# neofytr/LLMTokenizer

Measured on AMD Instinct MI355X. Metric: corpus MB/s per merge iter (train), 1 GiB synthetic corpus, higher is better.
Workload: dtype u32

## Files before the change

### llmtokenizer_amd/csrc/batch.hip

```cpp
#pragma once
#include "engine_common.h"

namespace bpeamd {

static_assert(TOPK == 64, "a wave holds a list, one entry per lane");
static_assert(BRB == 2 * (1024 / 64), "the select's 16 waves merge two partial lists each");
#ifndef BPE_SU
#define BPE_SU 1
#endif
#ifndef BPE_FORM_PRINT
#define BPE_FORM_PRINT 0
#endif
#ifndef BPE_RU
#define BPE_RU 4
#endif
#ifndef BPE_AU
#define BPE_AU 1
#endif
constexpr uint32_t AU = BPE_AU;
constexpr uint32_t SU = BPE_SU;
#ifndef BPE_RUN_THREAD_PAIRS
#define BPE_RUN_THREAD_PAIRS 16
#endif
constexpr uint32_t RUN_THREAD_PAIRS = BPE_RUN_THREAD_PAIRS, RUN_Q = 256;
// ... 819 lines not shown
        B->ticket = 0;
        B->k = k;
        B->z0 = 256 + md;
        nmem = k;
    }
    ts_mark(E, bi, BT_SEL_FOLD, false);
    __syncthreads();
    if (tid < nmem) E->tlen[256 + sc.merges_done + tid] = ctl[tid];
    for (uint32_t q = tid; q < CTL_SELECT_WORDS; q += blockDim.x) reinterpret_cast<uint32_t *>(Cg)[q] = scw[q];
    if (tid == 0) {
        Cg->hot_scanned = sc.hot_scanned;
        if (sc.err) Cg->err = sc.err;
    }
    for (uint32_t q = tid; q < BAT_HEAD_WORDS; q += blockDim.x) reinterpret_cast<uint32_t *>(Bg)[q] = sbw[q];
    for (uint32_t q = tid; q < clear_k * 4; q += blockDim.x) E->bvnl[q] = 0;
    if (xclr_k) {
        if (tid < XBH) E->xbat[tid] = 0;
        if (tid < 2 * xclr_k) E->xbat[XBH + (uint64_t)(tid >> 1) * xbat_member_words(xclr_w) + (tid & 1)] = 0;
    }
    if (tid == 0 && sc.stop != STOP_NONE && E->hprobe) {
        __hip_atomic_store(E->hprobe, sc.stop, __ATOMIC_RELAXED, __HIP_MEMORY_SCOPE_SYSTEM);
        __builtin_amdgcn_fence(__ATOMIC_RELEASE, "");
    }
    ts_mark(E, bi, BT_SEL_WB, false);
    ts_mark(E, bi, BT_SEL_OUT, false, true);
}

__device__ inline void rewrite_occ(const Eng *__restrict__ E, Ctl *__restrict__ C, Bat *__restrict__ B, uint32_t z,
                                   uint32_t la, uint32_t lb, uint32_t base, uint32_t obase, uint32_t elo, uint32_t ehi,
                                   uint32_t bidm, uint32_t nbm, uint64_t L1) {
    uint32_t *tok = E->tok;
    const uint64_t n = E->n0;
    const uint32_t tid = threadIdx.x;
    for (uint32_t e0 = elo + bidm * blockDim.x * RU; e0 < ehi; e0 += nbm * blockDim.x * RU) {
        uint32_t pos[RU];
        uint16_t tg[RU];
#pragma unroll
        for (uint32_t u = 0; u < RU; u++) {
            const uint32_t e = e0 + u * blockDim.x + tid;
            pos[u] = e < ehi ? E->ids_out[base + e] : 0u;
            tg[u] = e < ehi ? E->btag[base + e] : (uint16_t)0;
        }
#pragma unroll
        for (uint32_t u = 0; u < RU; u++) {
            const uint32_t e = e0 + u * blockDim.x + tid;
            if (e >= ehi) continue;
            const uint64_t i = pos[u], j = i + la, kq = j + lb;
            tok[i] = z;
            if (j < n) {
                if (kq - 1 - i > E->end_max) B->ra_err = 5;
                if (kq - 1 == j) {
                    tok[j] = end_code(kq - 1 - i);
                } else {
                    tok[j] = HOLE;
                    if (kq - 1 < n) tok[kq - 1] = end_code(kq - 1 - i);
                }
                if (j == L1) C->L1new = (uint32_t)i;
            }
            E->occ[obase + e] = (uint32_t)i;
            E->occnb[obase + e] = tg[u];
        }
    }
}

__device__ __attribute__((always_inline)) inline void bat_rewrite(const Eng *__restrict__ E, Ctl *__restrict__ C, Bat *__restrict__ B) {
    __shared__ uint32_t sz[BK], sla[BK], slb[BK], sR[BK], slo[BK], ssb[BK], spre[BK + 1], ablk[BK + 1];
    __shared__ uint32_t sk, stop_, am, last;
    const uint32_t tid = threadIdx.x, lane = tid & 63;
    const uint32_t nA = gridDim.x - BRB, bid = blockIdx.x - BRB;
    if (tid < 64) {
        const uint32_t k = aload(&B->ra_k);
        uint32_t R[NBK], lo[NBK], nb[NBK], nbp[NBK];
        unsigned long long tot = 0;
#pragma unroll
        for (uint32_t b = 0; b < NBK; b++) {
            const uint32_t q = 64 * b + lane;
            const bool in = q < k;
            R[b] = in ? B->ra_R[q] : 0u;
            lo[b] = in ? B->ra_lo[q] : 0u;
            tot += R[b] - lo[b];
        }
        tot = wave_sum(tot);
#pragma unroll
        for (uint32_t b = 0; b < NBK; b++) {
            const uint32_t q = 64 * b + lane;
            nb[b] = q < k ? 1 + (uint32_t)(tot ? (uint64_t)(nA - k) * (R[b] - lo[b]) / tot : 0) : 0;
            nbp[b] = nb[b];
        }
// ... 211 lines not shown
__device__ inline uint32_t tok_at_b(const uint32_t *__restrict__ tok, const BHalo &H, int64_t p, int64_t n) {
    if (p < 0) return SH && p >= -3 ? get3(H.HL, (uint32_t)(-1 - p)) : HOLE;
    if (p >= n) return SH && p - n < 3 ? get3(H.HR, (uint32_t)(p - n)) : HOLE;
    return tok[p];
}

template <bool SH>
__device__ inline uint32_t cover_of(const uint32_t *__restrict__ tok, const RoleTab &rt, const BHalo &H, uint32_t p,
                                    int64_t ps, int64_t n) {
    if (!(rt.get(p) >> 31)) return BK;
    const int64_t pps = v_left<SH>(tok, ps);
    const uint32_t pp = tok_at_b<SH>(tok, H, pps, n);
    const uint32_t mm = rt.member(pp, p);
    if (mm >= BK || pp != p) return mm;
    uint32_t L;
    if (SH && ps < 0) {
        L = H.hlr[mm];
    } else {
        L = 1;
        int64_t x = v_left<SH>(tok, ps);
        for (; x >= 0 && tok[x] == p; x = v_left<SH>(tok, x)) L++;
        if (SH && x < 0) L += H.hlr[mm];
    }
    return (L & 1) ? BK : mm;
}

template <bool SH>
__device__ inline uint32_t starts_of(const uint32_t *__restrict__ tok, const RoleTab &rt, const BHalo &H, uint32_t q,
                                     int64_t kq, int64_t n) {
    const uint32_t lq = rt.get(q) & 0x7FFFFFFFu;
    if (!lq) return BK;
    const int64_t kn = v_right(kq, lq, n);
    return rt.member(q, tok_at_b<SH>(tok, H, kn, n));
}

enum : uint32_t { GRF_LGO = 1, GRF_LEND = 2, GRF_IGO = 3, GRF_IEND = 4 };
__device__ void bscan_long_runs(const Eng *__restrict__ E, Bat *__restrict__ B, const uint32_t *__restrict__ tok,
                                const RoleTab &rt, const BHalo &H, int64_t n, uint32_t z0, uint32_t sgen) {
    const uint32_t lane = threadIdx.x & 63;
    const uint32_t ng = uni(min(aload(&B->gr_n), GRUN));
    const uint64_t stride = gr_stride(E->n0), maxch = stride - 1;
    auto flag_of = [&](uint32_t st) { return (sgen << 3) | st; };
    for (uint32_t gi = 0; gi < ng; gi++) {
        uint32_t ok = 1;
        if (lane == 0) {
            const unsigned long long t0 = wall_clock64();
            while (__hip_atomic_load(&B->gr_ready[gi], __ATOMIC_ACQUIRE, __HIP_MEMORY_SCOPE_AGENT) != sgen) {
                if (wall_clock64() - t0 > E->gr_wait) {
                    ok = 0;
                    B->ra_err = 11;
                    atomicAdd(&B->gr_tready, 1u);
                    break;
                }
                __builtin_amdgcn_s_sleep(1);
            }
        }
        if (!uni((uint32_t)__shfl((int)ok, 0))) return;
        const uint32_t mg = uni(aload(&B->gr_m[gi])), ag = uni(B->a[mg]), zg = z0 + mg;
        const int64_t c0 = uni(aload(&B->gr_c[gi])), lag = uni(E->tlen[ag]);
        uint32_t *occg = E->ids_out + B->sbase[mg];
        uint16_t *tagg = E->btag + B->sbase[mg];
        const uint32_t slice = B->sbase[mg + 1] - B->sbase[mg];
        uint32_t *flags = E->grflag + (uint64_t)gi * stride;
        auto pos = [&](int64_t l) -> int64_t { return c0 + l * lag; };
        auto tk = [&](int64_t l) -> uint32_t {
            const int64_t p = pos(l);
// ... 189 lines not shown
        if (SH) {
            Halo h;
            shard_halo(E->erec, E->nshards, E->shard, sa[tid], &h);
            H.hlr[tid] = h.hlrun;
            H.myi[tid] = h.myidx;
            if (tid == 0)
                for (int q = 0; q < 3; q++) {
                    H.HL[q] = h.HL[q];
                    H.HR[q] = h.HR[q];
                }
        }
    }
    const uint32_t a = sa[m], b = sb[m], z = z0 + m;
    const uint32_t la = E->tlen[a], lb = E->tlen[b];
    const uint32_t mode = B->mode[m], off = B->off[m], len = B->len[m];
    const uint32_t bid = blockIdx.x - B->blk0[m], nblk = B->blk0[m + 1] - B->blk0[m];
    const uint32_t sbase = B->sbase[m];
    uint32_t *occz = E->ids_out + sbase;
    uint16_t *tagz = E->btag + sbase;
    const uint32_t sslice = B->sbase[m + 1] - sbase;
#define STG(IDX, WHERE) if ((IDX) >= sslice) { B->ra_err = 12; } else
    uint32_t *Rm = &B->R[m];
    const int64_t n = (int64_t)E->n0;
    const uint32_t *__restrict__ tok = E->tok;
    const uint32_t want = mode == 2 ? a : b;
    const uint32_t lim = min(DENSE, z0 + k);
    for (uint32_t v = 0; v < 4; v++)
        for (uint32_t x = tid; x < lim; x += SCAN_T) s[v][x] = 0;
    __syncthreads();
    auto tok_at = [&](int64_t p) -> uint32_t { return tok_at_b<SH>(tok, H, p, n); };

    if (a != b) {
        static_assert(SU == 1 && BPE_WFLUSH, "the wave-driven candidate loop: one entry per lane per round");
        const uint32_t stride = nblk * SCAN_T;
        const uint32_t lane = tid & 63, wbase = (tid >> 6) * 64 * FR;
        uint32_t wcnt = 0, wocc = 0;
        uint32_t nent[SU];
        uint16_t ntg[SU];
        uint32_t eS = bid * SCAN_T + (tid & ~63u);
        auto load1 = [&](uint32_t s0, uint32_t &en, uint16_t &tg) {
            const uint32_t e = s0 + lane;
            en = 0;
            tg = 0xFFFFu;
            if (e < len) {
                en = mode == 0 ? E->plist[off + e] : E->occ[off + e];
                if (mode) tg = E->occnb[off + e];
            }
        };
        uint32_t pent = 0;
        uint16_t ptg = 0xFFFFu;
        auto advance = [&]() {
            eS += stride;
            if (SCAN_PD > 1) {
                nent[0] = pent;
                ntg[0] = ptg;
                if (eS + stride < len) load1(eS + stride, pent, ptg);
            } else if (eS < len) {
                load1(eS, nent[0], ntg[0]);
            }
        };
        auto flush = [&]() {
            __builtin_amdgcn_fence(__ATOMIC_RELEASE, "wavefront");
            __builtin_amdgcn_wave_barrier();
            uint32_t g = 0;
            if (lane == 0 && wcnt) g = atomicAdd(Rm, wcnt);
            g = __shfl(g, 0);
            for (uint32_t q = lane; q < wcnt; q += 64) {
                STG(g + q, "wflush") {
                occz[g + q] = list[wbase + q];
                tagz[g + q] = ltag[wbase + q];
                }
            }
            wocc += wcnt;
            wcnt = 0;
            __builtin_amdgcn_wave_barrier();
        };
        const bool cmp = mode != 0 && E->scan_compact != 0;
        const uint32_t tsh = mode == 2 ? 8u : 0u;
        uint32_t qpos = 0, qn = 0;
        load1(eS, nent[0], ntg[0]);
        if (SCAN_PD > 1) load1(eS + stride, pent, ptg);
        for (;;) {
            uint32_t ent[SU];
            uint16_t etg[SU];
            bool val[SU];
            if (!cmp) {
                if (eS >= len) break;
                val[0] = eS + lane < len;
                ent[0] = nent[0];
                etg[0] = ntg[0];
                advance();
            } else {
                while (eS < len) {
                    const bool pass = eS + lane < len && tag_ok(((uint32_t)ntg[0] >> tsh) & 0xFFu, want);
                    const unsigned long long M = __ballot(pass);
                    const uint32_t np = (uint32_t)__popcll(M);
                    if (qn + np > 64) break;
                    const uint32_t r = lane - qn;
                    const bool mine = lane >= qn && r < np;
                    const uint32_t pv = (uint32_t)__shfl((int)nent[0], (int)(mine ? kth_bit(M, r) : lane));
                    if (mine) qpos = pv;
                    qn += np;
                    advance();
                }
                if (qn == 0) break;
                val[0] = lane < qn;
                ent[0] = qpos;
                etg[0] = 0xFFFFu;
                qn = 0;
            }
            int64_t ii[SU], jj[SU];
            TokWin W[SU];
#pragma unroll
            for (uint32_t u = 0; u < SU; u++) {
                if (mode == 2) {
                    val[u] = val[u] && tag_ok(etg[u] >> 8, want);
                    jj[u] = ent[u];
                    ii[u] = 0;
                    if (val[u]) W[u] = tok_window(tok, jj[u]);
                } else {
                    val[u] = val[u] && (mode == 0 || tag_ok(etg[u] & 0xFFu, want));
                    ii[u] = ent[u];
                    jj[u] = ii[u] + la;
                    if (val[u]) W[u] = tok_window(tok, ii[u]);
                }
            }
            bool ok[SU];
            uint32_t tl[SU], tr[SU];
#pragma unroll
            for (uint32_t u = 0; u < SU; u++) {
                ok[u] = false;
                tl[u] = tr[u] = HOLE;
                if (!val[u]) continue;
                const int64_t j = jj[u];
                if (mode == 2) {
                    const uint32_t wl = j > 0 ? W[u].at(j - 1) : HOLE;
                    const int64_t i = j > 0 ? start_of_end<SH>(wl, j - 1) : -1;
                    ii[u] = i;
                    if (W[u].at(j) != b || i < 0) continue;
                    const uint32_t ti = W[u].has(i) ? W[u].at(i) : tok[i];
                    tl[u] = i > 0 ? (W[u].has(i - 1) ? W[u].at(i - 1) : tok[i - 1]) : HOLE;
                    const int64_t kk = j + lb;
                    tr[u] = kk < n ? (W[u].has(kk) ? W[u].at(kk) : tok[kk]) : HOLE;
                    ok[u] = ti == a;
                } else {
                    const int64_t i = ii[u], kk = j + lb;
                    const uint32_t t1 = j >= n ? HOLE : W[u].has(j) ? W[u].at(j) : tok[j];
                    tl[u] = i > 0 ? W[u].at(i - 1) : HOLE;
                    tr[u] = kk >= n ? HOLE : W[u].has(kk) ? W[u].at(kk) : tok[kk];
                    ok[u] = W[u].at(i) == a && t1 == b && j < n;
                }
            }
            int64_t ps[SU];
            uint32_t pv[SU];
#pragma unroll
            for (uint32_t u = 0; u < SU; u++) {
                const int64_t i = ii[u];
                ps[u] = i <= 0 ? -1 : start_of_end<SH>(tl[u], i - 1);
                pv[u] = ok[u] ? ((i > 0 && is_id(tl[u])) ? tl[u] : tok_at(ps[u])) : HOLE;
            }
#pragma unroll
            for (uint32_t u = 0; u < SU; u++) {
                const int64_t i = ii[u], j = jj[u];
                uint32_t lfin = HOLE, rfin = HOLE;
                if (ok[u]) {
                    const uint32_t p = pv[u];
                    lfin = p;
                    if (p != HOLE) {
                        const uint32_t cv = cover_of<SH>(tok, rt, H, p, ps[u], n);
                        if (cv < BK) {
                            lfin = z0 + cv;
                            mk_set(tadj, cv);
                            atomicAdd(&covc, 1u);
                        } else {
                            vadd_b(s, E, m, V_DL, p, gcnt);
                            vadd_b(s, E, m, V_IL, p, gcnt);
                        }
                    }
                    const int64_t kq = v_right(j, lb, n);
                    const uint32_t q = kq < n ? tr[u] : tok_at(kq);
                    rfin = q;
                    if (q != HOLE) {
                        const uint32_t st = starts_of<SH>(tok, rt, H, q, kq, n);
                        if (st < BK) {
                            rfin = z0 + st;
                            mk_set(tadj, st);
                        }
                        vadd_b(s, E, m, V_DR, q, gcnt);
                        vadd_b(s, E, m, V_IR, rfin, gcnt);
                    }
                }
                const unsigned long long om = __ballot(ok[u]);
                if (ok[u]) {
                    const uint32_t slot = wbase + wcnt + (uint32_t)__popcll(om & ((1ull << lane) - 1ull));
                    list[slot] = (uint32_t)i;
                    ltag[slot] = nb_tag(lfin, rfin);
                }
                wcnt += (uint32_t)__popcll(om);
            }
            if (wcnt + 64 > 64 * FR) flush();
        }
        if (wcnt) flush();
        if (lane == 0 && wocc) atomicAdd(&bRs, wocc);
    } else {
        for (uint32_t e0 = bid * SCAN_T; e0 < len; e0 += nblk * SCAN_T) {
            const uint32_t e = e0 + tid;
            int64_t i = 0;
            bool ok = false;
            if (e >= len) {
            } else if (mode == 2) {
                const int64_t j = E->occ[off + e];
                if (tag_ok(E->occnb[off + e] >> 8, want) && tok[j] == b) {
                    i = v_left<SH>(tok, j);
                    ok = i >= 0 && tok[i] == a;
                }
            } else {
                i = (mode == 0) ? E->plist[off + e] : E->occ[off + e];
                ok = (mode == 0 || tag_ok(E->occnb[off + e] & 0xFFu, want)) && tok[i] == a && i + la < n &&
                     tok[i + la] == b;
            }
            const int64_t ps = ok ? v_left<SH>(tok, i) : -1;
            const uint32_t p = ok ? tok_at(ps) : HOLE;
            const uint32_t cv = (ok && p != HOLE && p != a) ? cover_of<SH>(tok, rt, H, p, ps, n) : BK;
            if (cv < BK) {
                atomicAdd(&covc, 1u);
                mk_set(tadj, cv);
// ... 941 lines not shown
```

### llmtokenizer_amd/csrc/encode.hip

```cpp

namespace bpeamd {

__device__ inline void enc_desc(const Eng *E, uint32_t u, uint32_t v, uint32_t z, uint32_t *mode, uint32_t *off,
                                uint32_t *len) {
    *mode = 1;
    *off = 0;
    *len = 0;
    if (!(u < z && v < z)) return;
    if (u < 256 && v < 256) {
        const uint32_t ru = E->rank[u], rv = E->rank[v];
        if (ru != HOLE && rv != HOLE) {
            const uint32_t rk = ru * E->A + rv;
            *mode = 0;
            *off = E->poff[rk];
            *len = E->poff[rk + 1] - *off;
        }
        return;
    }
    if (u >= v) {
        *off = E->occ_off[u];
        *len = E->occ_len[u];
    } else {
        *mode = 2;
        *off = E->occ_off[v];
// ... 295 lines not shown
            C->counters[5] += spre[nb];
            C->counters[6]++;
            C->n_live -= spre[nb];
            const uint32_t xl = SH ? C->xleft : HOLE;
            if (xl != HOLE) {
                const uint64_t end = (uint64_t)xl + C->xleft_lb;
                if (end - 1 == xl) {
                    tok[xl] = MARKV;
                } else {
                    tok[xl] = HOLE;
                    if (end - 1 < n) tok[end - 1] = MARKV;
                }
                C->F1 = (uint32_t)(end < n ? end : n);
            }
        }
        __syncthreads();
        form_batch(E, C, E->eb + (p ^ 1), C->merges_done, occ_base + spre[nb]);
        return;
    }
    const uint32_t total = sseg[nb];
    const uint32_t *scratch = E->ids_out;
    const uint32_t nw = gridDim.x - 1;
    const uint64_t L1 = SH ? C->L1 : 0;
    for (uint32_t t = blockIdx.x * blockDim.x + tid; t < total; t += nw * blockDim.x) {
        const uint32_t m = seg_of(sseg, nb, t);
        const uint32_t q = t - sseg[m];
        if (q >= sR[m]) continue;
        const uint64_t i = scratch[t];
        const uint64_t j = i + sla[m], k = j + slb[m];
        tok[i] = sz[m];
        if (!SH || j < n) {
            if (k - 1 - i > E->end_max) C->err = 5;
            if (k - 1 == j) {
                tok[j] = end_code(k - 1 - i);
            } else {
                tok[j] = HOLE;
                if (!SH || k - 1 < n) tok[k - 1] = end_code(k - 1 - i);
            }
            if (SH && j == L1) C->L1new = (uint32_t)i;
        }
        E->occ[occ_base + spre[m] + q] = (uint32_t)i;
    }
}

template <bool SH>
__global__ __launch_bounds__(256) void k_link_batch(const Eng *__restrict__ E, const Ctl *__restrict__ C) {
    if (C->stop) return;
    const EncBatch *B = E->eb + C->ebp;
    const uint32_t nb = B->nbg;
    __shared__ uint32_t sseg[BMAX + 1], sz[BMAX], sR[BMAX], spre[BMAX + 1];
    const uint32_t tid = threadIdx.x;
    for (uint32_t m = tid; m <= nb; m += blockDim.x) sseg[m] = B->seg[m];
    for (uint32_t m = tid; m < nb; m += blockDim.x) {
        sz[m] = B->z[m];
        sR[m] = B->R[m];
    }
    __syncthreads();
    block_exscan256(sR, spre, nb);
    const uint32_t total = sseg[nb], occ_base = B->occ_base;
    const int64_t n = (int64_t)E->n0;
    const uint32_t *tok = E->tok;
    for (uint32_t t = blockIdx.x * blockDim.x + tid; t < total; t += gridDim.x * blockDim.x) {
        const uint32_t m = seg_of(sseg, nb, t);
        const uint32_t q = t - sseg[m];
        if (q >= sR[m]) continue;
        const uint32_t e = occ_base + spre[m] + q;
        const int64_t i = E->occ[e];
        const int64_t ps = v_left<SH>(tok, i);
        const int64_t k = i + E->tlen[sz[m]];
        E->occnb[e] = nb_tag(ps >= 0 ? tok[ps] : HOLE, k < n ? tok[k] : HOLE);
// ... 10 lines not shown
```

### llmtokenizer_amd/csrc/engine.hip

```cpp
#include <hip/hip_runtime.h>
#include <fcntl.h>
#include <unistd.h>
#include <cerrno>

#include <algorithm>
#include <chrono>
#include <cstdio>
#include <cstdlib>
#include <cstring>
#include <string>
#include <thread>
#include <vector>
#include <unordered_map>

#include <rocprim/rocprim.hpp>

#include "../../include/bpe_gpu.h"
#include "kernels.hip"
#include "batch.hip"
#include "encode.hip"
#include "encode_win.hip"
#include "encode_docs.hip"
#include "split.hip"
#include "train_split.hip"
// ... 437 lines not shown
    if (r) {
        c->zpend.clear();
        return r;
    }
    return 0;
}

int setup_run_body(bpe_gpu_ctx *c, uint32_t mcap, bool encode) {
    free_train(c);
    if (!encode) c->split_ready = false;
    Eng &h = c->h;
    h.n0 = c->n0;
    h.mcap = mcap;
    h.vcap = 256 + mcap;
    h.encode = encode ? 1 : 0;
    h.fast = c->fast || c->sharded;
    h.sharded = c->sharded;
    h.shard = c->shard;
    h.nshards = c->nshards;
    const uint64_t n0 = c->n0;
    int r;
    if ((r = dalloc(c, &h.tok, n0 + 8, false))) return r;
    if ((r = dalloc(c, &h.tlen, h.vcap))) return r;
    if ((r = dalloc(c, &h.rank, 256))) return r;
    if ((r = dalloc(c, &h.plist, n0, false))) return r;
    const uint64_t slack = c->sharded ? std::max<uint64_t>((uint64_t)mcap + 64, n0 / 16) : 0;
    const uint64_t occ_n = (n0 + slack + 2) & ~1ull;
    if ((r = dalloc(c, &h.occ, occ_n + n0, false))) return r;
    h.ids_out = h.occ + occ_n;
    if ((r = dalloc(c, &h.occnb, occ_n, false))) return r;
    h.xfused = c->sharded && c->xfused && !encode;
    h.end_max = END_MAX;
    if (const char *t = getenv("BPE_END_MAX")) h.end_max = std::min<uint64_t>(END_MAX, std::max(1ll, atoll(t)));
    h.track_ub = 1;
    if (const char *t = getenv("BPE_TRACK")) h.track_ub = (uint32_t)std::min(2, std::max(0, atoi(t)));
    h.light_wait = 100000000ull;
    if (const char *t = getenv("BPE_LIGHT_WAIT_TICKS")) h.light_wait = strtoull(t, nullptr, 10);
    h.xtimeout = c->xtimeout;
    h.xstride = (uint32_t)(((4ull * h.vcap + 2) + 63) & ~63ull);
    if (c->sharded) {
        if ((r = dalloc(c, &h.xbuf, 2ull * h.xstride))) return r;
        if ((r = dalloc(c, &h.myrec, EDGE_WORDS))) return r;
        if ((r = dalloc(c, &h.erec, (size_t)EDGE_WORDS * c->nshards))) return r;
    } else {
        h.xbuf = h.myrec = h.erec = nullptr;
    }
    if ((r = dalloc(c, &h.occ_off, h.vcap))) return r;
    if ((r = dalloc(c, &h.occ_len, h.vcap))) return r;
    if ((r = dalloc(c, &h.merges, 2ull * std::max<uint32_t>(mcap, 1)))) return r;
    for (int p = 0; p < 2; p++) {
        for (int v = 0; v < 4; v++) {
            if ((r = dalloc(c, &h.vec[p][v], encode ? 1 : std::max<uint32_t>(h.vcap, DENSE)))) return r;
            if ((r = dalloc(c, &h.vlist[p][v], encode ? 1 : h.vcap, false))) return r;
        }
        if ((r = dalloc(c, &h.vnl[p], 4))) return r;
    }
    if ((r = dalloc(c, &h.vecd, encode ? 1 : (size_t)2 * REPL * 4 * DENSE))) return r;
    if ((r = dalloc(c, &h.scan_tend, STAMPS))) return r;
    h.dbgts = nullptr;
    h.dbg_form = (uint32_t)getenv_int("BPE_DEBUG_FORM", 0);
    h.prefix_apply = (uint32_t)(getenv_int("BPE_PREFIX", 1) != 0);
    {
        int khz = 0;
        (void)hipDeviceGetAttribute(&khz, hipDeviceAttributeWallClockRate, c->dev);
        const int us = getenv_int("BPE_RW_HOLD_US", 0);
        h.rw_hold = (uint32_t)std::max(0, us) * (uint32_t)std::max(1, khz / 1000);
// ... 3164 lines not shown
```

### llmtokenizer_amd/csrc/engine_common.h

```cpp
#pragma once
#include <hip/hip_runtime.h>
#include <stddef.h>
#include <stdint.h>

namespace bpeamd {

constexpr uint32_t HOLE = 0xFFFFFFFFu;
constexpr uint32_t END_FLAG = 0x80000000u;
constexpr uint32_t MARKV = 0xFFFFFFFEu;
constexpr uint64_t END_MAX = 0x7FFFFFFDull;
__host__ __device__ inline bool is_id(uint32_t v) { return v < END_FLAG; }
__host__ __device__ inline uint32_t end_code(uint64_t d) { return END_FLAG | (uint32_t)d; }
#ifndef BPE_DENSE
#define BPE_DENSE 8192
#endif
constexpr uint32_t DENSE = BPE_DENSE;
#ifndef BPE_REPL
#define BPE_REPL 8
#endif
constexpr uint32_t REPL = BPE_REPL;
constexpr uint32_t NTHR = 16;
constexpr uint64_t CHUNK = 65536;
constexpr uint64_t DYN_LIMIT = CHUNK * NTHR;
constexpr uint64_t TRACK_LIMIT = 2 * DYN_LIMIT;
constexpr uint64_t TRACK_MIN_N = 4096;
constexpr uint64_t MERGED_B0 = 65536;
constexpr uint64_t THREAD_B0 = 256;
constexpr uint32_t L1W = 1024;
constexpr uint32_t L2W = 256;
constexpr uint32_t EDGE_WORDS = 16;
constexpr uint32_t TS_SLOTS = 16384;
enum { TS_K1_IN = 0, TS_K1_RESCAN, TS_K1_SCAN, TS_K2_IN, TS_K2_SELECT, TS_K2_APPLY_A, TS_K2_APPLY_B, TS_K1_LASTIN,
       TS_S_CAND, TS_S_LIST, TS_S_DELTA, TS_B_DVAL, TS_B_TABLE, TS_B_MARKS, TS_B_PROBE, TS_B_COUNT, TS_K1_CLEARED,
       TS_SPARE0, TS_SPARE1, TS_SPARE2, TS_SPARE3, TS_SPARE4, TS_SPARE5, TS_SPARE6, TS_SPARE7, TS_SPARE8, TS_N };

enum { V_DL = 0, V_DR = 1, V_IL = 2, V_IR = 3 };

enum : uint32_t {
    STOP_NONE = 0,
    STOP_DONE = 1,
    STOP_CAP = 2,
    STOP_EVENT = 3,
    STOP_GROW = 4,
    STOP_ERROR = 5,
    STOP_ENC_END = 6,
// ... 180 lines not shown
    const uint32_t *enc_pairs;
    uint32_t n_enc;
    EncBatch *eb;
    uint32_t hot;
    uint32_t hot_parts;
    uint32_t hot_target;
    uint32_t relist_stale;
    uint32_t *hot_slot;
    uint32_t *hot_hist;
    unsigned long long *hotp_best, *hotp_key, *hotp_v2, *hotp_k2;
    uint32_t *hotp_tie;
    uint32_t batch;
    uint32_t skip_on;
    uint32_t scan_compact;
    uint32_t scan_occd;
    uint32_t skg_exp;
    uint32_t nlists;
    uint32_t tie_up;
    uint32_t crate_pct;
    uint32_t lose_retry;
    uint32_t bvs;
    Bat *bat;
    uint16_t *btag;
    uint32_t *bvecd;
    uint32_t *bvec;
    uint32_t *bvlist;
    uint32_t *bvnl;
    uint32_t *xbat;
    uint32_t *grflag;
    unsigned long long gr_wait;
    uint32_t *xsp_out, *xsp_in;
    uint32_t xsp_cap, xsp_stride;
    uint64_t end_max;
    uint32_t track_ub;
    unsigned long long light_wait;
    unsigned long long *lkey, *lfirst;
    uint64_t lcap;
    unsigned long long *mlog;
    uint64_t mlog_cap;
};
constexpr uint32_t MLOG_WORDS = 5;
constexpr uint64_t MLOG_MAX = 1ull << 20;

struct Ctl {
    uint32_t a, b, z, stop;
    uint32_t merges_done, parity, R, occ_top;
    uint32_t cand_mode, cand_off, cand_len, stop_z;
    uint32_t nl2, full, event, ties;
    unsigned long long n_live;
    unsigned long long D;
    unsigned long long B;
    unsigned long long W;
    uint32_t edge, wslot, pad0, pad1;
    unsigned long long Bcur[NTHR];
    unsigned long long Bstart[NTHR];
    unsigned long long Bfin[NTHR];
    uint32_t Dt[NTHR];
    uint32_t follows[NTHR];
    uint32_t last_c[NTHR];
    unsigned long long stat_n;
    unsigned long long counters[12];
    unsigned long long scan_t0;
    unsigned long long scan_ticks;
    unsigned long long scan_launches;
    uint32_t sa, sb, s_mode, s_off;
    uint32_t s_len, spec, sRp[2];
// ... 166 lines not shown
```

### llmtokenizer_amd/csrc/kernels.hip

```cpp
#include "engine_common.h"
#include "p2p.hip"

namespace bpeamd {

__device__ inline uint32_t lane_id() { return __lane_id(); }

__device__ inline uint32_t aload(const uint32_t *p) {
    return __hip_atomic_load(p, __ATOMIC_RELAXED, __HIP_MEMORY_SCOPE_AGENT);
}
__device__ inline void astore(uint32_t *p, uint32_t v) {
    __hip_atomic_store(p, v, __ATOMIC_RELAXED, __HIP_MEMORY_SCOPE_AGENT);
}
__device__ inline unsigned long long aload64(const unsigned long long *p) {
    return __hip_atomic_load(p, __ATOMIC_RELAXED, __HIP_MEMORY_SCOPE_AGENT);
}

__device__ inline uint32_t wave_append(bool pred, uint32_t *counter) {
    unsigned long long m = __ballot(pred);
    if (m == 0) return 0;
    uint32_t lane = lane_id();
    uint32_t leader = __ffsll(m) - 1;
    uint32_t base = 0;
    if (lane == leader) base = atomicAdd(counter, (uint32_t)__popcll(m));
    base = __shfl(base, leader);
// ... 38 lines not shown
            atomicOr(&C->err, P2P_ERR_BIT);
            break;
        }
        __builtin_amdgcn_s_sleep(1);
    }
}

struct LazyHalo {
    const Eng *E;
    Ctl *C;
    uint32_t a;
    bool wait;
    bool ready;
    Halo h;
    __device__ inline const Halo &get() {
        if (!ready) {
            if (wait) {
                wait_records(E, C);
                shard_halo_ld(E->erec, E->nshards, E->shard, a, &h, [](const uint32_t *q) { return aload(q); });
            } else {
                shard_halo(E->erec, E->nshards, E->shard, a, &h);
            }
            ready = true;
        }
        return h;
    }
};

template <bool SH, typename HaloT>
__device__ inline uint32_t id_at(const uint32_t *__restrict__ tok, HaloT &h, int64_t p, int64_t n) {
    if (p < 0) return SH && p >= -3 ? get3(h.get().HL, (uint32_t)(-1 - p)) : HOLE;
    if (p >= n) return SH && p - n < 3 ? get3(h.get().HR, (uint32_t)(p - n)) : HOLE;
    return tok[p];
}

template <bool SH = true>
__device__ inline int64_t start_of_end(uint32_t v, int64_t e) {
    if (is_id(v)) return e;
    if (SH && v == MARKV) return -1;
    const int64_t d = v & ~END_FLAG;
    if (!SH) return e - d;
    return d > e ? -1 : e - d;
}

template <bool SH = true>
__device__ inline int64_t v_left(const uint32_t *__restrict__ tok, int64_t p) {
    if (p <= 0) return p - 1;
    return start_of_end<SH>(tok[p - 1], p - 1);
}

__device__ inline int64_t v_right(int64_t p, uint32_t len, int64_t n) {
    if (p >= n) return p + 1;
    const int64_t q = p + len;
    return q >= n ? n : q;
}

constexpr uint32_t SCAN_T = 1024;

struct TokWin {
    uint4 w0, w1;
    int64_t base;
    __device__ inline bool has(int64_t x) const { return x >= base && x < base + 8; }
    __device__ inline uint32_t at(int64_t x) const {
        const uint32_t k = (uint32_t)(x - base);
        const uint4 w = k < 4 ? w0 : w1;
        const uint32_t r = k & 3;
        return r == 0 ? w.x : r == 1 ? w.y : r == 2 ? w.z : w.w;
    }
};

__device__ inline TokWin tok_window(const uint32_t *__restrict__ tok, int64_t i) {
    TokWin W;
    W.base = (i > 0 ? i - 1 : 0) & ~3ll;
    const uint4 *p = reinterpret_cast<const uint4 *>(tok + W.base);
    W.w0 = p[0];
// ... 135 lines not shown
        bool ok = false;
        int64_t i = 0, j = 0;
        uint32_t tl = HOLE, tr = HOLE;
        if (e < len) {
            if (mode == 2) {
                j = E->occ[off + e];
                if (tag_ok(E->occnb[off + e] >> 8, want) && tok[j] == b) {
                    i = v_left<SH>(tok, j);
                    ok = i >= 0 && tok[i] == a;
                    if (ok) {
                        tl = i > 0 ? tok[i - 1] : HOLE;
                        tr = j + lb < n ? tok[j + lb] : HOLE;
                    }
                }
            } else {
                i = (mode == 0) ? E->plist[off + e] : E->occ[off + e];
                if (mode == 0 || tag_ok(E->occnb[off + e] & 0xFFu, want)) {
                    j = i + la;
                    const TokWin W = tok_window(tok, i);
                    const int64_t kk = j + lb;
                    const uint32_t t0 = W.at(i);
                    const uint32_t t1 = j >= n ? HOLE : W.has(j) ? W.at(j) : tok[j];
                    tl = i > 0 ? W.at(i - 1) : HOLE;
                    tr = kk >= n ? HOLE : W.has(kk) ? W.at(kk) : tok[kk];
                    ok = t0 == a && t1 == b && j < n;
                }
            }
        }
        if (a != b) {
            const uint32_t slot = wave_append(ok, &lcount);
            if (ok) {
                list[slot] = (uint32_t)i;
                const int64_t ps = i == 0 ? -1 : start_of_end<SH>(tl, i - 1);
                const uint32_t p = (i > 0 && is_id(tl)) ? tl : id_at<SH>(tok, h, ps, n);
                bool cov = false;
                if (p != HOLE) {
                    if (p == b) cov = id_at<SH>(tok, h, v_left<SH>(tok, ps), n) == a;
                    if (!cov && count) {
                        vadd<SH>(s, E, P, V_DL, p);
                        vadd<SH>(s, E, P, V_IL, p);
                    }
                }
                const int64_t k = v_right(j, lb, n);
                const uint32_t q = k < n ? tr : id_at<SH>(tok, h, k, n);
                bool nocc = false;
                if (q != HOLE) {
                    nocc = q == a && id_at<SH>(tok, h, v_right(k, la, n), n) == b;
                    if (count) {
                        vadd<SH>(s, E, P, V_DR, q);
                        vadd<SH>(s, E, P, V_IR, nocc ? z : q);
                    }
                }
                ltag[slot] = nb_tag(cov ? z : p, nocc ? z : q);
            }
        } else if (ok) {
            const int64_t ps = v_left<SH>(tok, i);
            const uint32_t p = id_at<SH>(tok, h, ps, n);
            bool start = true, left = p != HOLE;
            int64_t pos = i;
            if (p == a) {
                start = ps < 0;
                left = false;
                if (SH && (h.get().hlrun & 1)) pos = j;
            }
            for (uint32_t m = 0; start; m++) {
                const int64_t jj = pos + la;
                if (jj >= n || tok[jj] != a) break;
// ... 201 lines not shown
    if (valid) {
        if (u < 256 && v < 256) {
            const uint32_t ru = rank[u], rv = rank[v];
            if (ru != HOLE && rv != HOLE) {
                const uint32_t rk = ru * E->A + rv;
                mode = 0;
                off = poff[rk];
                len = poff[rk + 1] - off;
            }
        } else if (u >= v) {
            mode = 1; off = E->occ_off[u]; len = E->occ_len[u];
        } else {
            mode = 2; off = E->occ_off[v]; len = E->occ_len[v];
        }
    }
    *mode_o = mode;
    *off_o = off;
    *len_o = len;
}

constexpr uint32_t MARK_CAP = 1024;

template <bool UNDO>
__device__ inline void apply_body(const Eng *__restrict__ E, Ctl *__restrict__ C, const Snap &S, uint32_t bid,
                                  uint32_t nblk, uint32_t roleA_blocks, const P2P *__restrict__ X = nullptr) {
    const uint32_t a = S.a, b = S.b, z = S.z, R = S.R, P = S.parity;
    if (bid < roleA_blocks) {
        const uint32_t la = E->tlen[a], lb = E->tlen[b];
        const uint32_t *occz = E->occ + S.occ_top;
        uint32_t *tok = E->tok;
        const uint64_t n = E->n0;
        const bool sh = E->sharded;
        const uint64_t L1 = C->L1;
        for (uint32_t e = bid * blockDim.x + threadIdx.x; e < R; e += roleA_blocks * blockDim.x) {
            const uint64_t i = occz[e];
            const uint64_t j = i + la, k = j + lb;
            if (UNDO) {
                tok[i] = a;
                if (j < n) {
                    tok[j] = b;
                    if (lb > 1 && k - 1 < n) tok[k - 1] = end_code(lb - 1);
                }
                continue;
            }
            tok[i] = z;
            if (j < n) {
                if (k - 1 - i > E->end_max) C->err = 5;
                if (k - 1 == j) {
                    tok[j] = end_code(k - 1 - i);
                } else {
                    tok[j] = HOLE;
                    if (k - 1 < n) tok[k - 1] = end_code(k - 1 - i);
                }
                if (sh && j == L1) C->L1new = (uint32_t)i;
            }
        }
        if (!UNDO && bid == 0 && threadIdx.x == 0) {
            E->occ_off[z] = S.occ_top;
            E->occ_len[z] = R;
            C->pend[P] = 1;
            if (E->spec_on) E->tlen[z] = (a < z && b < z) ? la + lb : 1;
            const uint32_t xl = sh ? C->xleft : HOLE;
            if (xl != HOLE) {
                const uint64_t end = (uint64_t)xl + lb;
                if (end - 1 == xl) {
                    tok[xl] = MARKV;
                } else {
                    tok[xl] = HOLE;
                    if (end - 1 < n) tok[end - 1] = MARKV;
                }
                C->F1 = (uint32_t)(end < n ? end : n);
            }
            if (sh) C->erec_ready = 0;
        }
        if (UNDO && sh && bid == 0 && threadIdx.x == 0) {
            const uint32_t xl = C->xleft;
            if (xl != HOLE) {
                tok[xl] = b;
                const uint64_t end = (uint64_t)xl + lb;
                if (lb > 1 && end - 1 < n) tok[end - 1] = end_code(lb - 1);
                C->F1 = xl;
            }
            C->L1new = HOLE;
            C->erec_ready = 1;
        }
        return;
    }
    if (E->encode) return;
    const uint32_t nB = nblk - roleA_blocks;
    const uint32_t stride = nB * blockDim.x;
    uint32_t *const *lst = E->vlist[P];
    const bool sh = E->sharded;
    const uint32_t W = sh ? E->vcap : min(DENSE, E->vcap);
    uint32_t nl[4];
    for (int v = 0; v < 4; v++) nl[v] = sh ? 0 : E->vnl[P][v];
    const uint32_t dense_end = 1 + 4 * W;
    const uint32_t total = dense_end + nl[0] + nl[1] + nl[2] + nl[3];
    const uint32_t *xbP = sh ? xbufp(E, P) : nullptr;
    uint32_t XW = 1, xc0 = 0;
    if (sh && X) {
        const uint32_t seq = C->nx_seq0;
        const unsigned long long t0 = wall_clock64();
        if (threadIdx.x < X->W) p2p_wait(X, X->mb[X->rank] + MB_FLAG0 + 16 * threadIdx.x, seq, t0);
        __syncthreads();
        XW = X->W;
        xc0 = X->c0;
        xbP = X->mb[X->rank] + MB_DATA0 + (uint64_t)(seq & 1u) * XW * xc0;
    }
    uint32_t Rg = R;
    if (sh) {
        Rg = 0;
        for (uint32_t r = 0; r < XW; r++) Rg += xld(X, xbP + (uint64_t)r * xc0 + 4 * E->vcap);
    }
// ... 2537 lines not shown
        for (uint64_t p = sP[t] + g0; p < sP[t + 1]; p += gs) {
            const uint32_t x = E->tok[p];
            if (!is_id(x)) continue;
            const uint64_t q = p + E->tlen[x];
            if (q >= n0) continue;
            bool fresh = false;
            const int64_t s = light_slot(E, lkey48(t, x, E->tok[q]), gen, true, &fresh);
            if (s < 0) {
                bad = 1;
                continue;
            }
            if (fresh) atomicAdd(&cnt[t], 1u);
            atomicMin(&E->lfirst[s], ((unsigned long long)(0xFFFFu - gen) << 48) | p);
        }
    }
    __syncthreads();
    if (tid < NTHR && cnt[tid]) atomicAdd(&C->ldt[tid], cnt[tid]);
    if (tid == 0 && bad) atomicOr(&C->light_mask, 1u << 31);
    __threadfence();
    __syncthreads();
    if (tid == 0) last = atomicAdd(&C->lticket, 1u) == nblk - 1;
    __syncthreads();
    if (!last || tid >= 64) return;
    __threadfence();
    const uint32_t t = tid;
    const uint32_t lm = __hip_atomic_load(&C->light_mask, __ATOMIC_RELAXED, __HIP_MEMORY_SCOPE_AGENT);
    if (lm >> 31) {
        if (t == 0) C->stat_need = 1;
        return;
    }
    if (t < NTHR && ((mask >> t) & 1u)) {
        auto start_of = [&](uint64_t e) -> uint64_t {
            const uint32_t w = E->tok[e];
            return is_id(w) ? e : e - (w & ~END_FLAG);
        };
        uint64_t lp = start_of((uint64_t)sP[t + 1] - 1);
        if (t == NTHR - 1) lp = start_of(lp - 1);
        const uint32_t u = E->tok[lp], v = E->tok[lp + E->tlen[u]];
        bool fr = false;
        const int64_t s = light_slot(E, lkey48(t, u, v), gen, false, &fr);
        const unsigned long long f =
            s >= 0 ? __hip_atomic_load(&E->lfirst[s], __ATOMIC_RELAXED, __HIP_MEMORY_SCOPE_AGENT) : ~0ull;
        const uint32_t follows = s >= 0 && (f & LKEY_MASK) != lp;
        const uint32_t Dt = __hip_atomic_load(&C->ldt[t], __ATOMIC_RELAXED, __HIP_MEMORY_SCOPE_AGENT);
        const uint64_t Bf = thread_cascade(C->Bstart[t], Dt, follows);
        C->Bfin[t] = Bf;
        C->Bcur[t] = Bf;
        C->tUB[t] = Dt;
    }
    if (t == 0) {
        C->stat_need = 0;
        C->track_light++;
    }
}

__global__ __launch_bounds__(1024) void k_stat_light(const Eng *__restrict__ E, Ctl *__restrict__ C) {
    if (C->stop || C->stat_need != 2) return;
    light_body(E, C, blockIdx.x, gridDim.x);
}

__global__ void k_synth(uint8_t *__restrict__ out, uint64_t n, uint64_t seed, uint64_t off) {
    for (uint64_t i = (uint64_t)blockIdx.x * blockDim.x + threadIdx.x; i < n; i += (uint64_t)gridDim.x * blockDim.x) {
        uint64_t z = seed + (off + i + 1) * 0x9E3779B97F4A7C15ull;
        z = (z ^ (z >> 30)) * 0xBF58476D1CE4E5B9ull;
        z = (z ^ (z >> 27)) * 0x94D049BB133111EBull;
        z ^= z >> 31;
        out[i] = (uint8_t)(32 + (((z >> 32) * 95ull) >> 32));
// ... 114 lines not shown
```

Baseline: 126.0 million.

## Pack token id into end codes and add a register-window fast path to the scan

End markers now store the merged token id alongside the distance to the start, so the left neighbour's id can be read directly from the end word instead of chasing back to the start position. The candidate scan loop is restructured into a fast path that resolves neighbour ids, cover and starts from a vector window plus a few prefetched words. A wave falls back to the old dependent global loads only when some lane cannot resolve from registers. Loads are also made branchless with clamped indices, scalar-uniform loop bounds and global address-space casts. In exchange, the maximum encodable end distance is halved, and rewrite and decode paths must use the new encoding consistently.

```diff
diff --git a/llmtokenizer_amd/csrc/batch.hip b/llmtokenizer_amd/csrc/batch.hip
--- a/llmtokenizer_amd/csrc/batch.hip
+++ b/llmtokenizer_amd/csrc/batch.hip
@@ -875,6 +875,7 @@
     uint32_t *tok = E->tok;
     const uint64_t n = E->n0;
     const uint32_t tid = threadIdx.x;
+    const uint32_t eid = E->end_id_dist;
     for (uint32_t e0 = elo + bidm * blockDim.x * RU; e0 < ehi; e0 += nbm * blockDim.x * RU) {
         uint32_t pos[RU];
         uint16_t tg[RU];
@@ -893,10 +894,10 @@
             if (j < n) {
                 if (kq - 1 - i > E->end_max) B->ra_err = 5;
                 if (kq - 1 == j) {
-                    tok[j] = end_code(kq - 1 - i);
+                    tok[j] = end_code(kq - 1 - i, z, eid);
                 } else {
                     tok[j] = HOLE;
-                    if (kq - 1 < n) tok[kq - 1] = end_code(kq - 1 - i);
+                    if (kq - 1 < n) tok[kq - 1] = end_code(kq - 1 - i, z, eid);
                 }
                 if (j == L1) C->L1new = (uint32_t)i;
             }
@@ -1174,6 +1175,27 @@
     if (!lq) return BK;
     const int64_t kn = v_right(kq, lq, n);
     return rt.member(q, tok_at_b<SH>(tok, H, kn, n));
+}
+
+#define BPE_GLOBAL_AS __attribute__((address_space(1)))
+typedef uint32_t u32x4_g __attribute__((ext_vector_type(4)));
+__device__ __forceinline__ uint32_t gload(const uint32_t *p) { return *(const BPE_GLOBAL_AS uint32_t *)p; }
+__device__ __forceinline__ uint16_t gload(const uint16_t *p) { return *(const BPE_GLOBAL_AS uint16_t *)p; }
+__device__ __forceinline__ TokWin tok_window_g(const uint32_t *tok, int64_t i) {
+    TokWin W;
+    W.base = (i > 0 ? i - 1 : 0) & ~3ll;
+    const BPE_GLOBAL_AS u32x4_g *p = (const BPE_GLOBAL_AS u32x4_g *)(tok + W.base);
+    const u32x4_g lo = p[0], hi = p[1];
+    W.w0 = make_uint4(lo.x, lo.y, lo.z, lo.w);
+    W.w1 = make_uint4(hi.x, hi.y, hi.z, hi.w);
+    return W;
+}
+
+__device__ __forceinline__ bool round_word(const TokWin &W, int64_t x, int64_t pl, uint32_t xl, int64_t pr, uint32_t xr,
+                                           int64_t pj, uint32_t xj, int64_t pk, uint32_t xk, uint32_t &v) {
+    const bool hw = W.has(x), hl = x == pl, hr = x == pr, hj = x == pj, hk = x == pk;
+    v = hw ? W.at(x) : hl ? xl : hr ? xr : hj ? xj : xk;
+    return hw || hl || hr || hj || hk;
 }
 
 enum : uint32_t { GRF_LGO = 1, GRF_LEND = 2, GRF_IGO = 3, GRF_IEND = 4 };
@@ -1429,20 +1451,23 @@
 
     if (a != b) {
         static_assert(SU == 1 && BPE_WFLUSH, "the wave-driven candidate loop: one entry per lane per round");
-        const uint32_t stride = nblk * SCAN_T;
+        const uint32_t ulen = __builtin_amdgcn_readfirstlane(len);
+        const uint32_t stride = __builtin_amdgcn_readfirstlane(nblk * SCAN_T);
         const uint32_t lane = tid & 63, wbase = (tid >> 6) * 64 * FR;
         uint32_t wcnt = 0, wocc = 0;
         uint32_t nent[SU];
         uint16_t ntg[SU];
-        uint32_t eS = bid * SCAN_T + (tid & ~63u);
+        uint32_t eS = __builtin_amdgcn_readfirstlane(bid * SCAN_T + (tid & ~63u));
+        const uint32_t *ents = (mode == 0 ? E->plist : E->occ) + off;
+        const uint16_t *etags = E->occnb + off;
+        const uint32_t umode = __builtin_amdgcn_readfirstlane(mode);
+        const uint32_t ula = __builtin_amdgcn_readfirstlane(la), ulb = __builtin_amdgcn_readfirstlane(lb);
+        const uint32_t elast = ulen ? ulen - 1 : 0;
         auto load1 = [&](uint32_t s0, uint32_t &en, uint16_t &tg) {
-            const uint32_t e = s0 + lane;
-            en = 0;
+            const uint32_t e = min(s0 + lane, elast);
+            en = gload(ents + e);
             tg = 0xFFFFu;
-            if (e < len) {
-                en = mode == 0 ? E->plist[off + e] : E->occ[off + e];
-                if (mode) tg = E->occnb[off + e];
-            }
+            if (umode) tg = gload(etags + e);
         };
         uint32_t pent = 0;
         uint16_t ptg = 0xFFFFu;
@@ -1451,8 +1476,8 @@
             if (SCAN_PD > 1) {
                 nent[0] = pent;
                 ntg[0] = ptg;
-                if (eS + stride < len) load1(eS + stride, pent, ptg);
-            } else if (eS < len) {
+                if (eS + stride < ulen) load1(eS + stride, pent, ptg);
+            } else {
                 load1(eS, nent[0], ntg[0]);
             }
         };
@@ -1472,6 +1497,7 @@
             wcnt = 0;
             __builtin_amdgcn_wave_barrier();
         };
+        const bool fj = ula > 3, fk = ula + ulb > 3, fr = ula + ulb > 2;
         const bool cmp = mode != 0 && E->scan_compact != 0;
         const uint32_t tsh = mode == 2 ? 8u : 0u;
         uint32_t qpos = 0, qn = 0;
@@ -1482,14 +1508,14 @@
             uint16_t etg[SU];
             bool val[SU];
             if (!cmp) {
-                if (eS >= len) break;
-                val[0] = eS + lane < len;
+                if (eS >= ulen) break;
+                val[0] = eS + lane < ulen;
                 ent[0] = nent[0];
                 etg[0] = ntg[0];
                 advance();
             } else {
-                while (eS < len) {
-                    const bool pass = eS + lane < len && tag_ok(((uint32_t)ntg[0] >> tsh) & 0xFFu, want);
+                while (eS < ulen) {
+                    const bool pass = eS + lane < ulen && tag_ok(((uint32_t)ntg[0] >> tsh) & 0xFFu, want);
                     const unsigned long long M = __ballot(pass);
                     const uint32_t np = (uint32_t)__popcll(M);
                     if (qn + np > 64) break;
@@ -1506,65 +1532,107 @@
                 etg[0] = 0xFFFFu;
                 qn = 0;
             }
-            int64_t ii[SU], jj[SU];
-            TokWin W[SU];
-#pragma unroll
-            for (uint32_t u = 0; u < SU; u++) {
-                if (mode == 2) {
-                    val[u] = val[u] && tag_ok(etg[u] >> 8, want);
-                    jj[u] = ent[u];
-                    ii[u] = 0;
-                    if (val[u]) W[u] = tok_window(tok, jj[u]);
-                } else {
-                    val[u] = val[u] && (mode == 0 || tag_ok(etg[u] & 0xFFu, want));
-                    ii[u] = ent[u];
-                    jj[u] = ii[u] + la;
-                    if (val[u]) W[u] = tok_window(tok, ii[u]);
-                }
-            }
-            bool ok[SU];
-            uint32_t tl[SU], tr[SU];
-#pragma unroll
-            for (uint32_t u = 0; u < SU; u++) {
-                ok[u] = false;
-                tl[u] = tr[u] = HOLE;
-                if (!val[u]) continue;
-                const int64_t j = jj[u];
-                if (mode == 2) {
-                    const uint32_t wl = j > 0 ? W[u].at(j - 1) : HOLE;
-                    const int64_t i = j > 0 ? start_of_end<SH>(wl, j - 1) : -1;
-                    ii[u] = i;
-                    if (W[u].at(j) != b || i < 0) continue;
-                    const uint32_t ti = W[u].has(i) ? W[u].at(i) : tok[i];
-                    tl[u] = i > 0 ? (W[u].has(i - 1) ? W[u].at(i - 1) : tok[i - 1]) : HOLE;
-                    const int64_t kk = j + lb;
-                    tr[u] = kk < n ? (W[u].has(kk) ? W[u].at(kk) : tok[kk]) : HOLE;
-                    ok[u] = ti == a;
-                } else {
-                    const int64_t i = ii[u], kk = j + lb;
-                    const uint32_t t1 = j >= n ? HOLE : W[u].has(j) ? W[u].at(j) : tok[j];
-                    tl[u] = i > 0 ? W[u].at(i - 1) : HOLE;
-                    tr[u] = kk >= n ? HOLE : W[u].has(kk) ? W[u].at(kk) : tok[kk];
-                    ok[u] = W[u].at(i) == a && t1 == b && j < n;
-                }
-            }
-            int64_t ps[SU];
-            uint32_t pv[SU];
-#pragma unroll
-            for (uint32_t u = 0; u < SU; u++) {
-                const int64_t i = ii[u];
-                ps[u] = i <= 0 ? -1 : start_of_end<SH>(tl[u], i - 1);
-                pv[u] = ok[u] ? ((i > 0 && is_id(tl[u])) ? tl[u] : tok_at(ps[u])) : HOLE;
-            }
-#pragma unroll
-            for (uint32_t u = 0; u < SU; u++) {
-                const int64_t i = ii[u], j = jj[u];
+            const bool m2 = umode == 2;
+            const bool v0 = val[0] && (m2 ? tag_ok(etg[0] >> 8, want) : (umode == 0 || tag_ok(etg[0] & 0xFFu, want)));
+            const int64_t e0 = min((int64_t)ent[0], n - 1);
+            int64_t i = m2 ? 0 : e0;
+            const int64_t j = m2 ? e0 : e0 + ula, kk = j + ulb;
+            const TokWin W = tok_window_g(tok, e0);
+            uint32_t xl = HOLE, xr = HOLE, xj = HOLE, xk = HOLE;
+            if (!m2) {
+                xl = gload(tok + (e0 >= 2 ? e0 - 2 : 0));
+                if (fr) xr = gload(tok + min(kk + 1, n - 1));
+                if (fj) xj = gload(tok + min(j, n - 1));
+                if (fk) xk = gload(tok + min(kk, n - 1));
+            }
+            const int64_t pl = e0 - 2, pr = fr ? kk + 1 : -1, pj = fj ? j : -1, pk = fk ? kk : -1;
+#define reg(X, V) round_word(W, (X), pl, xl, pr, xr, pj, xj, pk, xk, (V))
+            bool ok = false, need = v0 && m2;
+            uint32_t p = HOLE, q = HOLE, cv = BK, st = BK;
+            if (v0 && !m2) {
+                uint32_t t1 = HOLE;
+                if (j < n && !reg(j, t1)) need = true;
+                ok = !need && W.at(i) == a && t1 == b && j < n;
+                if (ok) {
+                    if (i == 0) {
+                        need = SH;
+                    } else {
+                        const uint32_t tl = W.at(i - 1);
+                        const int64_t ps = start_of_end<SH>(tl, i - 1);
+                        p = is_id(tl) ? tl : end_id(tl);
+                        if (p == HOLE) {
+                            need = true;
+                        } else if (rt.get(p) >> 31) {
+                            uint32_t w = HOLE;
+                            if (ps <= 0 || !reg(ps - 1, w)) {
+                                need = true;
+                            } else {
+                                const uint32_t pp = is_id(w) ? w : end_id(w);
+                                const uint32_t mm = pp == HOLE ? BK : rt.member(pp, p);
+                                if (pp == HOLE || (mm < BK && pp == p)) need = true;
+                                else cv = mm;
+                            }
+                        }
+                    }
+                    if (kk >= n) {
+                        need = need || SH;
+                    } else if (!reg(kk, q)) {
+                        need = true;
+                    } else if (q != HOLE) {
+                        const uint32_t lq = rt.get(q) & 0x7FFFFFFFu;
+                        if (lq) {
+                            const int64_t kn = kk + lq;
+                            uint32_t w = HOLE;
+                            if (kn >= n) {
+                                if (SH) need = true;
+                                else st = rt.member(q, HOLE);
+                            } else if (!reg(kn, w)) {
+                                need = true;
+                            } else {
+                                st = rt.member(q, w);
+                            }
+                        }
+                    }
+                }
+            }
+#undef reg
+            if (__ballot(need)) {
+                if (need) {
+                    ok = false;
+                    p = q = HOLE;
+                    cv = st = BK;
+                    uint32_t tl = HOLE, tr = HOLE;
+                    if (m2) {
+                        const uint32_t wl = j > 0 ? W.at(j - 1) : HOLE;
+                        i = j > 0 ? start_of_end<SH>(wl, j - 1) : -1;
+                        if (W.at(j) == b && i >= 0) {
+                            const uint32_t ti = W.has(i) ? W.at(i) : tok[i];
+                            tl = i > 0 ? (W.has(i - 1) ? W.at(i - 1) : tok[i - 1]) : HOLE;
+                            tr = kk < n ? (W.has(kk) ? W.at(kk) : tok[kk]) : HOLE;
+                            ok = ti == a;
+                        }
+                    } else {
+                        const uint32_t t1 = j >= n ? HOLE : W.has(j) ? W.at(j) : tok[j];
+                        tl = i > 0 ? W.at(i - 1) : HOLE;
+                        tr = kk >= n ? HOLE : W.has(kk) ? W.at(kk) : tok[kk];
+                        ok = W.at(i) == a && t1 == b && j < n;
+                    }
+                    if (ok) {
+                        const int64_t ps = i <= 0 ? -1 : start_of_end<SH>(tl, i - 1);
+                        const uint32_t pe = i > 0 ? (is_id(tl) ? tl : end_id(tl)) : HOLE;
+                        p = pe != HOLE ? pe : tok_at(ps);
+                        if (p != HOLE) cv = cover_of<SH>(tok, rt, H, p, ps, n);
+                        const int64_t kq = v_right(j, lb, n);
+                        q = kq < n ? tr : tok_at(kq);
+                        if (q != HOLE) st = starts_of<SH>(tok, rt, H, q, kq, n);
+                    }
+                }
+            }
+            {
                 uint32_t lfin = HOLE, rfin = HOLE;
-                if (ok[u]) {
-                    const uint32_t p = pv[u];
+                if (ok) {
                     lfin = p;
                     if (p != HOLE) {
-                        const uint32_t cv = cover_of<SH>(tok, rt, H, p, ps[u], n);
                         if (cv < BK) {
                             lfin = z0 + cv;
                             mk_set(tadj, cv);
@@ -1574,11 +1642,8 @@
                             vadd_b(s, E, m, V_IL, p, gcnt);
                         }
                     }
-                    const int64_t kq = v_right(j, lb, n);
-                    const uint32_t q = kq < n ? tr[u] : tok_at(kq);
                     rfin = q;
                     if (q != HOLE) {
-                        const uint32_t st = starts_of<SH>(tok, rt, H, q, kq, n);
                         if (st < BK) {
                             rfin = z0 + st;
                             mk_set(tadj, st);
@@ -1587,8 +1652,8 @@
                         vadd_b(s, E, m, V_IR, rfin, gcnt);
                     }
                 }
-                const unsigned long long om = __ballot(ok[u]);
-                if (ok[u]) {
+                const unsigned long long om = __ballot(ok);
+                if (ok) {
                     const uint32_t slot = wbase + wcnt + (uint32_t)__popcll(om & ((1ull << lane) - 1ull));
                     list[slot] = (uint32_t)i;
                     ltag[slot] = nb_tag(lfin, rfin);
diff --git a/llmtokenizer_amd/csrc/encode.hip b/llmtokenizer_amd/csrc/encode.hip
--- a/llmtokenizer_amd/csrc/encode.hip
+++ b/llmtokenizer_amd/csrc/encode.hip
@@ -351,10 +351,10 @@
         if (!SH || j < n) {
             if (k - 1 - i > E->end_max) C->err = 5;
             if (k - 1 == j) {
-                tok[j] = end_code(k - 1 - i);
+                tok[j] = end_code(k - 1 - i, sz[m], E->end_id_dist);
             } else {
                 tok[j] = HOLE;
-                if (!SH || k - 1 < n) tok[k - 1] = end_code(k - 1 - i);
+                if (!SH || k - 1 < n) tok[k - 1] = end_code(k - 1 - i, sz[m], E->end_id_dist);
             }
             if (SH && j == L1) C->L1new = (uint32_t)i;
         }
diff --git a/llmtokenizer_amd/csrc/engine.hip b/llmtokenizer_amd/csrc/engine.hip
--- a/llmtokenizer_amd/csrc/engine.hip
+++ b/llmtokenizer_amd/csrc/engine.hip
@@ -493,6 +493,10 @@
     h.xfused = c->sharded && c->xfused && !encode;
     h.end_max = END_MAX;
     if (const char *t = getenv("BPE_END_MAX")) h.end_max = std::min<uint64_t>(END_MAX, std::max(1ll, atoll(t)));
+    h.end_id_dist = END_ID_DIST;
+    if (const char *t = getenv("BPE_END_ID_DIST")) h.end_id_dist = (uint32_t)std::min<long long>(END_ID_DIST, std::max(0ll, atoll(t)));
+    if (const char *t = getenv("BPE_END_ID")) if (atoi(t) == 0) h.end_id_dist = 0;
+    h.end_pad = 0;
     h.track_ub = 1;
     if (const char *t = getenv("BPE_TRACK")) h.track_ub = (uint32_t)std::min(2, std::max(0, atoi(t)));
     h.light_wait = 100000000ull;
diff --git a/llmtokenizer_amd/csrc/engine_common.h b/llmtokenizer_amd/csrc/engine_common.h
--- a/llmtokenizer_amd/csrc/engine_common.h
+++ b/llmtokenizer_amd/csrc/engine_common.h
@@ -8,9 +8,32 @@
 constexpr uint32_t HOLE = 0xFFFFFFFFu;
 constexpr uint32_t END_FLAG = 0x80000000u;
 constexpr uint32_t MARKV = 0xFFFFFFFEu;
-constexpr uint64_t END_MAX = 0x7FFFFFFDull;
+constexpr uint32_t END_PLAIN = 0x40000000u;
+constexpr uint32_t END_ID_BITS = 18, END_DIST_BITS = 12;
+constexpr uint32_t END_ID_DIST = (1u << END_DIST_BITS) - 1;
+constexpr uint64_t END_MAX = 0x3FFFFFFDull;
+static_assert(END_ID_BITS + END_DIST_BITS == 30, "bits 0..29 of an end code");
+static_assert((END_FLAG | END_PLAIN | (uint32_t)END_MAX) < MARKV, "no end code is MARKV or HOLE");
 __host__ __device__ inline bool is_id(uint32_t v) { return v < END_FLAG; }
-__host__ __device__ inline uint32_t end_code(uint64_t d) { return END_FLAG | (uint32_t)d; }
+__host__ __device__ inline uint32_t end_code(uint64_t d, uint32_t id, uint32_t id_dist = END_ID_DIST) {
+    const uint32_t lim = id_dist < END_ID_DIST ? id_dist : END_ID_DIST;
+    if (d <= lim && id < (1u << END_ID_BITS)) return END_FLAG | (id << END_DIST_BITS) | (uint32_t)d;
+    return END_FLAG | END_PLAIN | (uint32_t)d;
+}
+__host__ __device__ inline uint32_t end_dist(uint32_t v) {
+    return (v & END_PLAIN) ? (v & (END_PLAIN - 1)) : (v & END_ID_DIST);
+}
+__host__ __device__ inline uint32_t end_id(uint32_t v) {
+    return (v & (END_FLAG | END_PLAIN)) == END_FLAG ? (v >> END_DIST_BITS) & ((1u << END_ID_BITS) - 1) : HOLE;
+}
+template <bool SH = true>
+__host__ __device__ inline int64_t start_of_end(uint32_t v, int64_t e) {
+    if (is_id(v)) return e;
+    if (SH && v == MARKV) return -1;
+    const int64_t d = end_dist(v);
+    if (!SH) return e - d;
+    return d > e ? -1 : e - d;
+}
 #ifndef BPE_DENSE
 #define BPE_DENSE 8192
 #endif
@@ -257,6 +280,7 @@
     uint32_t *xsp_out, *xsp_in;
     uint32_t xsp_cap, xsp_stride;
     uint64_t end_max;
+    uint32_t end_id_dist, end_pad;
     uint32_t track_ub;
     unsigned long long light_wait;
     unsigned long long *lkey, *lfirst;
diff --git a/llmtokenizer_amd/csrc/kernels.hip b/llmtokenizer_amd/csrc/kernels.hip
--- a/llmtokenizer_amd/csrc/kernels.hip
+++ b/llmtokenizer_amd/csrc/kernels.hip
@@ -94,15 +94,6 @@
     if (p < 0) return SH && p >= -3 ? get3(h.get().HL, (uint32_t)(-1 - p)) : HOLE;
     if (p >= n) return SH && p - n < 3 ? get3(h.get().HR, (uint32_t)(p - n)) : HOLE;
     return tok[p];
-}
-
-template <bool SH = true>
-__device__ inline int64_t start_of_end(uint32_t v, int64_t e) {
-    if (is_id(v)) return e;
-    if (SH && v == MARKV) return -1;
-    const int64_t d = v & ~END_FLAG;
-    if (!SH) return e - d;
-    return d > e ? -1 : e - d;
 }
 
 template <bool SH = true>
@@ -304,7 +295,8 @@
             if (ok) {
                 list[slot] = (uint32_t)i;
                 const int64_t ps = i == 0 ? -1 : start_of_end<SH>(tl, i - 1);
-                const uint32_t p = (i > 0 && is_id(tl)) ? tl : id_at<SH>(tok, h, ps, n);
+                const uint32_t pe = i > 0 ? (is_id(tl) ? tl : end_id(tl)) : HOLE;
+                const uint32_t p = pe != HOLE ? pe : id_at<SH>(tok, h, ps, n);
                 bool cov = false;
                 if (p != HOLE) {
                     if (p == b) cov = id_at<SH>(tok, h, v_left<SH>(tok, ps), n) == a;
@@ -572,6 +564,7 @@
         const uint64_t n = E->n0;
         const bool sh = E->sharded;
         const uint64_t L1 = C->L1;
+        const uint32_t eid = E->end_id_dist;
         for (uint32_t e = bid * blockDim.x + threadIdx.x; e < R; e += roleA_blocks * blockDim.x) {
             const uint64_t i = occz[e];
             const uint64_t j = i + la, k = j + lb;
@@ -579,7 +572,7 @@
                 tok[i] = a;
                 if (j < n) {
                     tok[j] = b;
-                    if (lb > 1 && k - 1 < n) tok[k - 1] = end_code(lb - 1);
+                    if (lb > 1 && k - 1 < n) tok[k - 1] = end_code(lb - 1, b, eid);
                 }
                 continue;
             }
@@ -587,10 +580,10 @@
             if (j < n) {
                 if (k - 1 - i > E->end_max) C->err = 5;
                 if (k - 1 == j) {
-                    tok[j] = end_code(k - 1 - i);
+                    tok[j] = end_code(k - 1 - i, z, eid);
                 } else {
                     tok[j] = HOLE;
-                    if (k - 1 < n) tok[k - 1] = end_code(k - 1 - i);
+                    if (k - 1 < n) tok[k - 1] = end_code(k - 1 - i, z, eid);
                 }
                 if (sh && j == L1) C->L1new = (uint32_t)i;
             }
@@ -618,7 +611,7 @@
             if (xl != HOLE) {
                 tok[xl] = b;
                 const uint64_t end = (uint64_t)xl + lb;
-                if (lb > 1 && end - 1 < n) tok[end - 1] = end_code(lb - 1);
+                if (lb > 1 && end - 1 < n) tok[end - 1] = end_code(lb - 1, b, eid);
                 C->F1 = xl;
             }
             C->L1new = HOLE;
@@ -3222,7 +3215,7 @@
     if (t < NTHR && ((mask >> t) & 1u)) {
         auto start_of = [&](uint64_t e) -> uint64_t {
             const uint32_t w = E->tok[e];
-            return is_id(w) ? e : e - (w & ~END_FLAG);
+            return is_id(w) ? e : e - end_dist(w);
         };
         uint64_t lp = start_of((uint64_t)sP[t + 1] - 1);
         if (t == NTHR - 1) lp = start_of(lp - 1);
```

New measurement: 128.7 million, median of 6. +2.2%, better.
